# CSB5/XNA_Basecaller

Hardware: NVIDIA B200
Metric: signal samples/sec basecalled (sup@v3.3 XNA) (higher is better)
Workload: dtype fp16

## Files before the change

xna_basecaller_b200/csrc/inproj_gemm.cu:

```cuda
#include <stdlib.h>

#include "xb_common.cuh"
#include "xb_ptx.cuh"
#include "xb_gemm.cuh"
#include "xb_head_epilogue.cuh"
#include "xb_exact_math.h"

using namespace xbptx;

namespace {

#ifdef XB_EXPERIMENTS
#define IP_CLK() clock64()
#else
#define IP_CLK() 0ll
#endif

constexpr int BM = 128, BNI = 64, BK = 64;
constexpr int KB = XB_FEATURES / BK;
constexpr int MAX_COLS = XB_GATES;
constexpr int KPS = 4;
constexpr int SPT = KB / KPS;
enum { IP_GATES = 0, IP_SCORES = 1 };
template <int EPI> struct IPCfg {
    static constexpr int STAGES = EPI == IP_GATES ? 6 : 4;
    static constexpr int SETS = EPI == IP_GATES ? 1 : 2;
    static constexpr int THREADS = (4 + 4 * SETS) * 32;
    static constexpr int STG_BYTES = EPI == IP_GATES ? 32 * (BNI * 2 + 16) : 32 * 81 * 4;
    static constexpr int SMEM_BYTES = STAGES * (KPS * BNI * BK * 2) + 4 * SETS * STG_BYTES + MAX_COLS * 4 + 1024  + 512 ;
};
constexpr int KBLOCK_BYTES = BNI * BK * 2;
constexpr int STAGE_BYTES = KPS * KBLOCK_BYTES;
constexpr int A_COLS = XB_FEATURES / 2;
constexpr int ROW_PITCH = BNI * 2 + 16;

struct IPParams {
    const uint16_t *x;
    const float *bias;
    void *out;
    int M;
    int NT;
    int n_valid, ldo;
    int n_base, expand;
    float scale, blank;
    int exp_out;
    int no_prefetch;
    long long *dbg;
};

template <int NB, bool FULL>
__device__ __forceinline__ void head_stage64(const float (&v)[BNI], uint32_t sr, int e0, int pos0, int ncols, float blank) {
#pragma unroll
    for (int jj = 0; jj < BNI; jj++) {
        if (FULL || jj < ncols) {
            const unsigned u = (unsigned)(e0 + jj);
            const unsigned g = u / NB;
            const uint32_t a = sr + 4u * (uint32_t)(pos0 + jj + (int)g);
            sts_f32(a, v[jj]);
            if (u - g * NB == 0) sts_f32(a - 4u, blank);
        }
    }
}
template <bool FULL>
__device__ __forceinline__ void head_stage64_dyn(const float (&v)[BNI], uint32_t sr, int nb, int e0, int pos0, int ncols, float blank) {
    int e = e0, o = pos0;
#pragma unroll
    for (int jj = 0; jj < BNI; jj++) {
        if (FULL || jj < ncols) {
            if (e == 0) sts_f32(sr + 4u * (uint32_t)(o - 1), blank);
            sts_f32(sr + 4u * (uint32_t)o, v[jj]);
            o++;
            if (++e == nb) { e = 0; o++; }
        }
    }
}

template <bool BF16, int EPI, bool XCP>
__global__ void __launch_bounds__(IPCfg<EPI>::THREADS, 1)
inproj_kernel(const __grid_constant__ CUtensorMap tmW, const __grid_constant__ CUtensorMap tmX, const IPParams p) {
    using X = xb16<BF16>;
    constexpr int STAGES = IPCfg<EPI>::STAGES, STG_BYTES = IPCfg<EPI>::STG_BYTES;
    const int NT = p.NT;
    extern __shared__ uint8_t smem_raw[];
    uint8_t *smem = reinterpret_cast<uint8_t *>((reinterpret_cast<uintptr_t>(smem_raw) + 1023) & ~uintptr_t(1023));
    uint8_t *stgbuf = smem + STAGES * STAGE_BYTES;
    float *sbias = reinterpret_cast<float *>(stgbuf + 4 * IPCfg<EPI>::SETS * STG_BYTES);
    uint64_t *full = reinterpret_cast<uint64_t *>(sbias + MAX_COLS);
    uint64_t *empty = full + STAGES;
    uint64_t *acc_full = empty + STAGES;
    uint64_t *acc_empty = acc_full + 2;
    uint64_t *a_ready = acc_empty + 2;
    uint32_t *tmem_holder = reinterpret_cast<uint32_t *>(a_ready + SPT);

    const int warp = __shfl_sync(0xffffffffu, (int)(threadIdx.x >> 5), 0), lane = threadIdx.x & 31;
    const int ntiles = (p.M + BM - 1) / BM;

    if (warp == 0 && lane == 0) {
        prefetch_tmap(&tmW);
        for (int s = 0; s < STAGES; s++) {
            mbar_init(&full[s], 1);
            mbar_init(&empty[s], 1);
        }
        for (int b = 0; b < 2; b++) {
            mbar_init(&acc_full[b], 1);
            mbar_init(&acc_empty[b], 4);
        }
        for (int ks = 0; ks < SPT; ks++) mbar_init(&a_ready[ks], 4);
        fence_barrier_init();
    }
    if (warp == 2) {
        tmem_alloc(tmem_holder, 512);
        tmem_relinquish();
    }
    for (int i = threadIdx.x; i < NT * BNI; i += IPCfg<EPI>::THREADS) sbias[i] = i < p.n_valid ? p.bias[i] : 0.0f;
    tc_fence_before();
    __syncthreads();
    tc_fence_after();
    const uint32_t tmem_base = *tmem_holder;

    if (warp == 0) {
        if (elect_one()) {
            uint32_t it = 0;
            for (int tile = blockIdx.x; tile < ntiles; tile += gridDim.x) {
                if (XCP)
                    for (int xs = 0; xs < KB / 2; xs++, it++) {
                        const int s = it % STAGES;
                        mbar_wait(&empty[s], ((it / STAGES) & 1) ^ 1);
                        mbar_expect_tx(&full[s], STAGE_BYTES);
                        tma_load_3d(smem + s * STAGE_BYTES, &tmX, &full[s], 0, tile * BM, xs * 2);
                    }
                for (int nt = 0; nt < NT; nt++)
                    for (int ks = 0; ks < SPT; ks++, it++) {
                        const int s = it % STAGES;
                        mbar_wait(&empty[s], ((it / STAGES) & 1) ^ 1);
                        mbar_expect_tx(&full[s], STAGE_BYTES);
                        tma_load_3d(smem + s * STAGE_BYTES, &tmW, &full[s], 0, nt * BNI, ks * KPS);
                    }
            }
        }
    } else if (warp == 1) {
        constexpr uint32_t idesc = umma_idesc_f16(BF16 ? 1u : 0u, BM, BNI);
        uint32_t it = 0, nit = 0, tit = 0;
        long long st_acc = 0, st_full = 0, st_issue = 0, st_a = 0, tt;
        const bool dbg = p.dbg && blockIdx.x == 0;
        for (int tile = blockIdx.x; tile < ntiles; tile += gridDim.x, tit++) {
            if (XCP) {
                tt = IP_CLK();
                for (int xs = 0; xs < KB / 2; xs++, it++) {
                    const int s = it % STAGES;
                    mbar_wait(&full[s], (it / STAGES) & 1);
                    tc_fence_after();
                    if (elect_one()) {
                        const uint64_t sdesc = umma_desc_sw128(smem_u32(smem + s * STAGE_BYTES));
#pragma unroll
                        for (int kk = 0; kk < 8; kk++)
                            tmem_cp_128x256b(tmem_base + (xs * 2) * (BK / 2) + kk * 8,
                                             sdesc + (uint64_t)(((kk >> 2) * (BM * BK * 2) + (kk & 3) * 32) >> 4));
                        mma_commit(&empty[s]);
                    }
                    __syncwarp();
                }
                st_a += IP_CLK() - tt;
            }
            for (int nt = 0; nt < NT; nt++, nit++) {
                const int buf = nit & 1;
                tt = IP_CLK();
                mbar_wait(&acc_empty[buf], ((nit >> 1) & 1) ^ 1);
                tc_fence_after();
                st_acc += IP_CLK() - tt;
                const uint32_t d = tmem_base + A_COLS + buf * BNI;
                for (int ks = 0; ks < SPT; ks++, it++) {
                    const int s = it % STAGES;
                    tt = IP_CLK();
                    mbar_wait(&full[s], (it / STAGES) & 1);
                    tc_fence_after();
                    st_full += IP_CLK() - tt;
                    if (!XCP && nt == 0) {
                        tt = IP_CLK();
                        mbar_wait(&a_ready[ks], tit & 1);
                        tc_fence_after();
                        st_a += IP_CLK() - tt;
                    }
                    tt = IP_CLK();
                    if (elect_one()) {
                        const uint64_t bdesc = umma_desc_sw128(smem_u32(smem + s * STAGE_BYTES));
                        const uint32_t a0 = tmem_base + ks * KPS * (BK / 2);
#pragma unroll
                        for (int kk = 0; kk < KPS * 4; kk++) {
                            const int kc = kk >> 2, k = kk & 3;
                            mma_f16_ts(d, a0 + kk * 8, bdesc + (uint64_t)((kc * KBLOCK_BYTES + k * 32) >> 4), idesc,
                                       (ks | kk) != 0);
                        }
                        mma_commit(&empty[s]);
                        if (ks == SPT - 1) mma_commit(&acc_full[buf]);
                    }
                    __syncwarp();
                    st_issue += IP_CLK() - tt;
                }
            }
        }
        if (dbg && lane == 0) { p.dbg[0] = st_acc; p.dbg[1] = st_full; p.dbg[2] = st_issue; p.dbg[3] = st_a; p.dbg[4] = tit; }
    } else if (warp >= 4) {
        constexpr int SETS = IPCfg<EPI>::SETS;
        const int set = (warp - 4) >> 2;
        const int q = warp & 3, r = q * 32 + lane;
        const uint32_t lane_base = tmem_base + ((uint32_t)(q * 32) << 16);
        uint8_t *stg = stgbuf + (set * 4 + q) * STG_BYTES;
        const uint32_t stg_s = smem_u32(stg);
        uint32_t nit = 0;
        bool pending = false;
        int pend_m0 = 0;

        auto epilogue = [&](int m0, int nt, uint32_t ni) {
            const int buf = ni & 1;
            uint32_t acc[BNI];
            {
                uint32_t a0[32], a1[32];
                tmem_ld_32x32b_x32(lane_base + A_COLS + buf * BNI, a0);
                tmem_ld_32x32b_x32(lane_base + A_COLS + buf * BNI + 32, a1);
                tmem_ld_wait();
#pragma unroll
                for (int i = 0; i < 32; i++) { acc[i] = a0[i]; acc[32 + i] = a1[i]; }
            }
            tc_fence_before();
            __syncwarp();
            if (lane == 0) mbar_arrive(&acc_empty[buf]);
            if constexpr (EPI == IP_GATES) {
                const float *bs = sbias + nt * BNI;
    #pragma unroll
                for (int j = 0; j < BNI / 8; j++) {
                    uint32_t pk[4];
    #pragma unroll
                    for (int e = 0; e < 4; e++)
                        pk[e] = X::pack(__uint_as_float(acc[8 * j + 2 * e]) + bs[8 * j + 2 * e],
                                        __uint_as_float(acc[8 * j + 2 * e + 1]) + bs[8 * j + 2 * e + 1]);
                    sts_v4(stg_s + lane * ROW_PITCH + j * 16, make_uint4(pk[0], pk[1], pk[2], pk[3]));
                }
                __syncwarp();
                const int sub = lane >> 3, l8 = lane & 7;
    #pragma unroll
                for (int rr = 0; rr < 32; rr += 4) {
                    const int mm = m0 + q * 32 + rr + sub;
                    if (mm < p.M)
                        reinterpret_cast<uint4 *>(reinterpret_cast<uint16_t *>(p.out) + (size_t)mm * p.ldo + nt * BNI)[l8] =
                            lds_v4(stg_s + (rr + sub) * ROW_PITCH + l8 * 16);
                }
            } else {
                constexpr int RS = 81;
                float *S = reinterpret_cast<float *>(stg);
// ... 42 lines not shown
                        for (int r = 0; r < 4; r++) {
                            const uint32_t a = sl + (uint32_t)((rr + r) * RS * 4);
                            w[r][0] = k0 ? lds_f32(a) : 0.0f;
                            w[r][1] = k1 ? lds_f32(a + 128) : 0.0f;
                            w[r][2] = k2 ? lds_f32(a + 256) : 0.0f;
                        }
#pragma unroll
                        for (int r = 0; r < 4; r++) {
                            const int mm = m0 + q * 32 + rr + r;
                            if (mm < p.M) {
                                float *o = obase + (size_t)mm * p.ldo;
                                if (k0) o[0] = w[r][0];
                                if (k1) o[32] = w[r][1];
                                if (k2) o[64] = w[r][2];
                            }
                        }
                    }
                    if (dbg) p.dbg[7] += IP_CLK() - te0;
                }
            }
            __syncwarp();
        };

        for (int tile = blockIdx.x; tile < ntiles || pending; tile += gridDim.x) {
            const bool valid = tile < ntiles;
            const int m0 = tile * BM;
            if (pending && ((!XCP && set == 0) || SETS == 1 || (int)((nit - 1) & 1) == set)) {
                mbar_wait(&acc_full[(nit - 1) & 1], ((nit - 1) >> 1) & 1);
                tc_fence_after();
            }
            const long long tl0 = IP_CLK();
            if (!XCP && valid && set == 0) {
                const int sub = lane >> 3, l8 = lane & 7;
                const int mrow0 = m0 + q * 32;
                constexpr int NBK = 2;
                static_assert(KPS == 2 * NBK && KB % KPS == 0, "one a_ready group = two rounds");
                uint4 ldA[NBK][8], ldB[NBK][8];
                auto issue = [&](uint4 (&ld)[NBK][8], int kb0) {
#pragma unroll
                    for (int b = 0; b < NBK; b++)
#pragma unroll
                        for (int i = 0; i < 8; i++) {
                            const int mm = mrow0 + 4 * i + sub;
                            ld[b][i] = (mm < p.M) ? __ldg(reinterpret_cast<const uint4 *>(p.x + (size_t)mm * XB_FEATURES + (kb0 + b) * BK) + l8)
                                                  : make_uint4(0, 0, 0, 0);
                        }
                };
                auto consume = [&](uint4 (&ld)[NBK][8], int kb0) {
#pragma unroll
                    for (int b = 0; b < NBK; b++) {
#pragma unroll
                        for (int i = 0; i < 8; i++)
                            sts_v4(stg_s + (4 * i + sub) * ROW_PITCH + l8 * 16, ld[b][i]);
                        __syncwarp();
                        uint32_t v[32];
#pragma unroll
                        for (int i = 0; i < 8; i++) {
                            const uint4 t4 = lds_v4(stg_s + lane * ROW_PITCH + i * 16);
                            v[4 * i] = t4.x; v[4 * i + 1] = t4.y; v[4 * i + 2] = t4.z; v[4 * i + 3] = t4.w;
                        }
                        __syncwarp();
                        tmem_st_32x32b_x32(lane_base + (kb0 + b) * (BK / 2), v);
                    }
                };
                issue(ldA, 0);
#pragma unroll 1
                for (int kb0 = 0; kb0 < KB; kb0 += KPS) {
                    issue(ldB, kb0 + NBK);
                    consume(ldA, kb0);
                    if (kb0 + KPS < KB) issue(ldA, kb0 + KPS);
                    consume(ldB, kb0 + NBK);
                    tmem_st_wait();
                    tc_fence_before();
                    __syncwarp();
                    if (lane == 0) mbar_arrive(&a_ready[kb0 / KPS]);
                }
            }
            if (p.dbg && blockIdx.x == 0 && warp == 4 && lane == 0) p.dbg[5] += IP_CLK() - tl0;
            for (int nt = -1; nt < (valid ? NT - 1 : 0); nt++) {
                int em0, ent;
                uint32_t eni;
                if (nt < 0) {
                    if (!pending || (SETS > 1 && (int)((nit - 1) & 1) != set)) continue;
                    em0 = pend_m0; ent = NT - 1; eni = nit - 1;
                } else {
                    if (SETS > 1 && (int)(nit & 1) != set) { nit++; continue; }
                    if (nt == (NT > 8 ? NT - 8 : 0) && !p.no_prefetch) {
                        const int mn = m0 + (int)gridDim.x * BM + r;
                        if (mn < p.M) {
                            const char *nx = reinterpret_cast<const char *>(p.x + (size_t)mn * XB_FEATURES);
#pragma unroll
                            for (int i = 0; i < 12; i++) asm volatile("prefetch.global.L2 [%0];" ::"l"(nx + i * 128));
                        }
                    }
                    mbar_wait(&acc_full[nit & 1], (nit >> 1) & 1);
                    tc_fence_after();
                    em0 = m0; ent = nt; eni = nit;
                    nit++;
                }
                epilogue(em0, ent, eni);
            }
            if (valid) {
                nit++;
                pend_m0 = m0;
            }
            pending = valid;
        }
    }
    tc_fence_before();
    __syncthreads();
    if (warp == 2) {
        tc_fence_after();
        tmem_dealloc(tmem_base, 512);
    }
}

}

template <int EPI>
static int ip_launch(xb_handle *h, const void *w, int w_rows, IPParams p, cudaStream_t s) {
    CUtensorMap tmW, tmX;
    if (int rc = xb_make_tmap_hview(h, &tmW, w, w_rows, BNI, KPS)) return rc;
    if (int rc = xb_make_tmap_hview(h, &tmX, p.x, (uint64_t)p.M, BM, 2)) return rc;
    p.NT = w_rows / BNI;
    p.dbg = nullptr;
    p.no_prefetch = 0;
#ifdef XB_EXPERIMENTS
    static const bool regload = getenv("XB_INPROJ_REGLOAD") != nullptr;
    p.no_prefetch = getenv("XB_INPROJ_NOPF") ? 1 : 0;
    if (getenv("XB_INPROJ_DEBUG")) {
        static long long *d = nullptr;
        if (!d) cudaMalloc(&d, 64);
        p.dbg = d;
    }
#endif
    const int ntiles = (p.M + BM - 1) / BM;
    const int grid = ntiles < h->num_sms ? ntiles : h->num_sms;
    constexpr int SMEM_BYTES = IPCfg<EPI>::SMEM_BYTES;
    static bool configured[4][64] = {};
    const int dv = h->device & 63;
    auto go = [&](auto kernel, int slot) -> int {
        if (!configured[slot][dv]) {
            XB_CUDA(h, cudaFuncSetAttribute(kernel, cudaFuncAttributeMaxDynamicSharedMemorySize, SMEM_BYTES));
            configured[slot][dv] = true;
        }
        kernel<<<grid, IPCfg<EPI>::THREADS, SMEM_BYTES, s>>>(tmW, tmX, p);
        return XB_OK;
    };
    int rc;
#ifdef XB_EXPERIMENTS
    if (regload) rc = go(inproj_kernel<false, EPI, false>, 2);
    else
#endif
    rc = go(inproj_kernel<false, EPI, true>, 3);
    if (rc) return rc;
    XB_LAUNCH_CHECK(h);
#ifdef XB_EXPERIMENTS
    if (p.dbg) {
        long long v[8];
        cudaDeviceSynchronize();
        cudaMemcpy(v, p.dbg, sizeof v, cudaMemcpyDeviceToHost);
        fprintf(stderr, "inproj MMA thread of CTA 0: %lld tiles; stall cycles: acc_empty %lld, full %lld, a_ready %lld; issue %lld; x-block load (warp 4) %lld; head epilogue stage %lld, stage+copy %lld\n", v[4], v[0], v[1], v[3], v[2], v[5], v[6], v[7]);
        cudaMemset(p.dbg, 0, 64);
    }
#endif
    return XB_OK;
}

int xb_inproj_launch(xb_handle *h, const void *x, const void *w_ih, const float *bias, void *gates, int M, cudaStream_t s) {
    IPParams p = {};
    p.x = reinterpret_cast<const uint16_t *>(x);
    p.bias = bias;
    p.out = gates;
    p.M = M;
    p.n_valid = XB_GATES; p.ldo = XB_GATES;
    return ip_launch<IP_GATES>(h, w_ih, XB_GATES, p, s);
}

int xb_head_astationary_launch(xb_handle *h, const void *x, const void *w, int w_rows, const float *bias, int head_rows,
                               float *scores, int ldo, int M, int exp_out, cudaStream_t s) {
    XB_REQUIRE(h, w_rows % BNI == 0 && w_rows <= MAX_COLS && head_rows <= w_rows, "head of %d rows unsupported", head_rows);
    IPParams p = {};
    p.x = reinterpret_cast<const uint16_t *>(x);
    p.bias = bias;
    p.out = scores;
// ... 8 lines not shown
```

xna_basecaller_b200/csrc/xb_api.cu:

```cuda
#include <stdarg.h>
#include <stdlib.h>
#include <string.h>

#include "xb_common.cuh"
#include "xb_gemm.cuh"

thread_local std::string xb_global_err;

int xb_fail(xb_handle *h, int code, const char *fmt, ...) {
    char buf[512];
    va_list ap;
    va_start(ap, fmt);
    vsnprintf(buf, sizeof buf, fmt, ap);
    va_end(ap);
    if (h) h->err = buf;
    xb_global_err = buf;
    return code;
}

int xb_conv12_im2col(xb_handle *h, const void *signal, int sig_dtype, int N, int L, cudaStream_t s);
int xb_lstm_recurrence_persistent(xb_handle *h, int layer, void *y_tnc, int T, int N, int reverse, cudaStream_t s, void *save = nullptr);
int xb_inproj_launch(xb_handle *h, const void *x, const void *w_ih, const float *bias, void *gates, int M, cudaStream_t s);
int xb_head_astationary_launch(xb_handle *h, const void *x, const void *w, int w_rows, const float *bias, int head_rows,
                               float *scores, int ldo, int M, int exp_out, cudaStream_t s);
int xb_preprocess_impl(xb_handle *h, const int16_t *raw, const int64_t *read_offset, const int32_t *read_len,
                       const double *scaling, const int32_t *offset, int n_reads, float *out, int32_t *out_len,
                       float *stats, cudaStream_t s);
int xb_ctc_loss_bwd_impl(xb_handle *h, const float *scores, int T, int N, const int32_t *targets, int Lmax,
                         const int32_t *lengths, int normalise, const float *grad_loss, float *alpha_ws, float *grad,
                         cudaStream_t s);
int xb_ctc_loss_impl(xb_handle *h, const float *scores, int T, int N, const int32_t *targets, int Lmax,
                     const int32_t *lengths, int normalise, float *loss, cudaStream_t s);
int xb_stitch_impl(xb_handle *h, const int8_t *rows, int T, const int32_t *chunk_first, const int32_t *chunk_count,
                   const int32_t *read_len, int n_reads, int chunksize, int overlap, int stride, int reverse, int8_t *out,
                   int out_stride, int32_t *out_len, cudaStream_t s);

void xb_train_free(xb_handle *h);
int xb_beam_search_impl(xb_handle *h, const float *scores, const float *beta, int T, int N, int beam_width, float beam_cut,
                        int8_t *seq, int8_t *qstring, int8_t *moves, int32_t *lens, cudaStream_t s);
int xb_onehot_edges(xb_handle *h, const int32_t *edges_nt, int T, int N, int S, float *post, cudaStream_t s);
int xb_gather_chunks_impl(xb_handle *h, const void *signal, int sig_dtype, const int64_t *read_offset,
                          const int32_t *read_len, const int32_t *chunk_read, const int32_t *chunk_start, int n_chunks,
                          int L, float *out, cudaStream_t s);

namespace {
// ... 132 lines not shown
    h->device = device;
    h->max_N = max_N;
    h->max_T = max_T;
    h->n_base = n_base;
    h->state_len = state_len;
    h->C = ipow(n_base, state_len);
    h->NZ = n_base + 1;
    h->flags = flags;
    h->bf16 = (flags & XB_FLAG_BF16) != 0;
    h->num_sms = prop.multiProcessorCount;
    strncpy(h->alphabet, alphabet, sizeof h->alphabet - 1);

    const size_t TN = (size_t)max_T * max_N, S = (size_t)h->C * h->NZ;
    int rc = XB_OK;
#define TRY(x) if (rc == XB_OK) rc = (x)
    const size_t VP = (size_t)((h->C + 31) / 32) * 32 + 4;
    TRY(dev_alloc(h, &h->alpha, (TN + max_N) * VP));
    TRY(dev_alloc(h, &h->bmax, (TN + max_N) * VP));
    TRY(dev_alloc(h, &h->lp, (TN + max_N) * VP));
    TRY(dev_alloc(h, &h->logz, (size_t)max_N));
    TRY(dev_alloc(h, &h->seq_dev, TN));
    TRY(dev_alloc(h, &h->lens_dev, (size_t)max_N));
    if (!(flags & XB_FLAG_NO_ENCODER)) {
        TRY(dev_alloc_bytes(h, &h->c2, TN * XB_CONV3_K * 2));
        TRY(dev_alloc_bytes(h, &h->act0, TN * XB_FEATURES * 2));
        TRY(dev_alloc_bytes(h, &h->act1, TN * XB_FEATURES * 2));
        TRY(dev_alloc_bytes(h, &h->gates, TN * XB_GATES * 2));
        TRY(dev_alloc(h, &h->cstate, (size_t)max_N * XB_FEATURES));
        TRY(dev_alloc(h, &h->scores, TN * S));
        TRY(dev_alloc_bytes(h, &h->signal_dev, TN * XB_STRIDE * sizeof(float)));
    }
#undef TRY
    if (rc != XB_OK) {
        xb_global_err = h->err;
        xb_destroy(h);
        return rc;
    }
    *out = h;
    return XB_OK;
}

int xb_destroy(xb_handle *h) {
    if (!h) return XB_OK;
    cudaSetDevice(h->device);
    void *ptrs[] = {h->conv1_w, h->conv1_b, h->conv2_w, h->conv2_b, h->conv3_w, h->conv3_b, h->head_w, h->head_b, h->c2,
                    h->act0, h->act1, h->gates, h->cstate, h->hzero, h->scores, h->signal_dev, h->seq_dev, h->lens_dev,
// ... 485 lines not shown
```

xna_basecaller_b200/csrc/xb_common.cuh:

```cuda
#pragma once

#include <cuda_runtime.h>
#include <cuda_fp16.h>
#include <cuda_bf16.h>
#include <cuda.h>
#include <stdint.h>
#include <stdio.h>
#include <string>
#include <vector>

#include "../../include/xna_basecaller.h"

#define XB_FEATURES 768
#define XB_GATES (4 * XB_FEATURES)
#define XB_STRIDE 5
#define XB_WINLEN 19
#define XB_C2_CH 16
#define XB_C2_HALO 9
#define XB_CONV3_K 320

struct xb_lstm_weights {
    void *w_ih = nullptr;
    void *w_hh = nullptr;
    float *bias = nullptr;
    void *w_ihT = nullptr;
    void *w_hhT = nullptr;
};

enum { XB_ST_CONV12 = 0, XB_ST_CONV3, XB_ST_INPROJ, XB_ST_LSTM_REC, XB_ST_HEAD, XB_ST_CRF_ALPHA, XB_ST_CRF_BACKWARD,
       XB_ST_CRF_VITERBI, XB_ST_TRAIN_BPTT, XB_ST_TRAIN_TRANSPOSE, XB_ST_TRAIN_WGRAD, XB_ST_TRAIN_XGRAD, XB_ST_TRAIN_HEAD_CONV,
       XB_ST_COUNT };

struct xb_prof_span { int stage; cudaEvent_t a, b; };

struct xb_handle {
    int device = 0;
    bool profiling = false;
    std::vector<xb_prof_span> spans;
    std::vector<cudaEvent_t> event_pool;
    int max_N = 0, max_T = 0;
    int n_base = 0, state_len = 0, C = 0, NZ = 0;
    int flags = 0;
    bool bf16 = false;
    int loaded = 0;
    char alphabet[16] = {0};
    int num_sms = 0;
    int64_t launches = 0;
    std::string err;

    float *conv1_w = nullptr, *conv1_b = nullptr, *conv2_w = nullptr, *conv2_b = nullptr;
    void *conv3_w = nullptr;
    float *conv3_b = nullptr;
    xb_lstm_weights lstm[5];
    void *head_w = nullptr;
    float *head_b = nullptr;
    int head_rows = 0, head_rows_padded = 0;
    float scale = 5.0f, blank_score = 2.0f;
    int expand_blanks = 1;

    void *c2 = nullptr;
    void *act0 = nullptr, *act1 = nullptr;
    void *gates = nullptr;
    float *cstate = nullptr;
    void *hzero = nullptr;
    float *scores = nullptr;
    void *signal_dev = nullptr;
    int8_t *seq_dev = nullptr;
    int32_t *lens_dev = nullptr;
    void *signal_dev2 = nullptr;
// ... 97 lines not shown
```

xna_basecaller_b200/csrc/xb_ptx.cuh:

```cuda
#pragma once
#include <cuda.h>
#include <stdint.h>

namespace xbptx {

__device__ __forceinline__ uint32_t smem_u32(const void *p) { return (uint32_t)__cvta_generic_to_shared(p); }

__device__ __forceinline__ bool elect_one() {
    uint32_t pred;
    asm volatile(
        "{\n\t.reg .pred P;\n\t.reg .b32 R;\n\t"
        "elect.sync R|P, 0xffffffff;\n\t"
        "selp.b32 %0, 1, 0, P;\n\t}"
        : "=r"(pred));
    return pred != 0;
}

__device__ __forceinline__ void mbar_init(uint64_t *bar, uint32_t count) {
    asm volatile("mbarrier.init.shared::cta.b64 [%0], %1;" ::"r"(smem_u32(bar)), "r"(count));
}
__device__ __forceinline__ void fence_barrier_init() { asm volatile("fence.mbarrier_init.release.cluster;" ::: "memory"); }
__device__ __forceinline__ void fence_proxy_async() { asm volatile("fence.proxy.async.shared::cta;" ::: "memory"); }
__device__ __forceinline__ void fence_proxy_async_all() { asm volatile("fence.proxy.async;" ::: "memory"); }
__device__ __forceinline__ void fence_proxy_async_global() { asm volatile("fence.proxy.async.global;" ::: "memory"); }
// ... 51 lines not shown
        "mbarrier.try_wait.parity.shared::cta.b64 P, [%1], %2;\n\t"
        "selp.b32 %0, 1, 0, P;\n\t}"
        : "=r"(ok)
        : "r"(smem_u32(bar)), "r"(parity)
        : "memory");
    return ok != 0;
}
__device__ __forceinline__ bool mbar_test_wait(uint64_t *bar, uint32_t parity) {
    uint32_t ok;
    asm volatile(
        "{\n\t.reg .pred P;\n\t"
        "mbarrier.test_wait.parity.shared::cta.b64 P, [%1], %2;\n\t"
        "selp.b32 %0, 1, 0, P;\n\t}"
        : "=r"(ok)
        : "r"(smem_u32(bar)), "r"(parity)
        : "memory");
    return ok != 0;
}
__device__ __forceinline__ void mbar_wait(uint64_t *bar, uint32_t parity) {
    while (!mbar_try_wait(bar, parity)) {
    }
}

__device__ __forceinline__ void prefetch_tmap(const CUtensorMap *m) {
    asm volatile("prefetch.tensormap [%0];" ::"l"(m) : "memory");
}
__device__ __forceinline__ void tma_load_2d(void *dst, const CUtensorMap *m, uint64_t *bar, int c0, int c1) {
    asm volatile(
        "cp.async.bulk.tensor.2d.shared::cluster.global.mbarrier::complete_tx::bytes [%0], [%1, {%3, %4}], [%2];"
        ::"r"(smem_u32(dst)), "l"(m), "r"(smem_u32(bar)), "r"(c0), "r"(c1)
        : "memory");
}
__device__ __forceinline__ void tma_load_3d(void *dst, const CUtensorMap *m, uint64_t *bar, int c0, int c1, int c2) {
    asm volatile(
        "cp.async.bulk.tensor.3d.shared::cluster.global.mbarrier::complete_tx::bytes [%0], [%1, {%3, %4, %5}], [%2];"
        ::"r"(smem_u32(dst)), "l"(m), "r"(smem_u32(bar)), "r"(c0), "r"(c1), "r"(c2)
        : "memory");
}

__device__ __forceinline__ void tma_store_2d(const CUtensorMap *m, uint32_t src_smem, int c0, int c1) {
    asm volatile("cp.async.bulk.tensor.2d.global.shared::cta.bulk_group [%0, {%2, %3}], [%1];"
                 ::"l"(m), "r"(src_smem), "r"(c0), "r"(c1) : "memory");
}
__device__ __forceinline__ void tma_load_4d(void *dst, const CUtensorMap *m, uint64_t *bar, int c0, int c1, int c2, int c3) {
    asm volatile(
        "cp.async.bulk.tensor.4d.shared::cluster.global.mbarrier::complete_tx::bytes [%0], [%1, {%3, %4, %5, %6}], [%2];"
        ::"r"(smem_u32(dst)), "l"(m), "r"(smem_u32(bar)), "r"(c0), "r"(c1), "r"(c2), "r"(c3)
        : "memory");
}
__device__ __forceinline__ void tma_store_4d(const CUtensorMap *m, uint32_t src_smem, int c0, int c1, int c2, int c3) {
    asm volatile("cp.async.bulk.tensor.4d.global.shared::cta.bulk_group [%0, {%2, %3, %4, %5}], [%1];"
                 ::"l"(m), "r"(src_smem), "r"(c0), "r"(c1), "r"(c2), "r"(c3) : "memory");
}
__device__ __forceinline__ void griddep_launch_dependents() { asm volatile("griddepcontrol.launch_dependents;" ::: "memory"); }
__device__ __forceinline__ void griddep_wait() { asm volatile("griddepcontrol.wait;" ::: "memory"); }
__device__ __forceinline__ void bulk_commit_group() { asm volatile("cp.async.bulk.commit_group;" ::: "memory"); }
__device__ __forceinline__ void bulk_wait_group0() { asm volatile("cp.async.bulk.wait_group 0;" ::: "memory"); }

__device__ __forceinline__ void tmem_alloc(uint32_t *holder_smem, uint32_t ncols) {
    asm volatile("tcgen05.alloc.cta_group::1.sync.aligned.shared::cta.b32 [%0], %1;" ::"r"(smem_u32(holder_smem)), "r"(ncols)
                 : "memory");
}
__device__ __forceinline__ void tmem_relinquish() {
    asm volatile("tcgen05.relinquish_alloc_permit.cta_group::1.sync.aligned;" ::: "memory");
}
__device__ __forceinline__ void tmem_dealloc(uint32_t taddr, uint32_t ncols) {
    asm volatile("tcgen05.dealloc.cta_group::1.sync.aligned.b32 %0, %1;" ::"r"(taddr), "r"(ncols) : "memory");
}
__device__ __forceinline__ void tc_fence_before() { asm volatile("tcgen05.fence::before_thread_sync;" ::: "memory"); }
__device__ __forceinline__ void tc_fence_after() { asm volatile("tcgen05.fence::after_thread_sync;" ::: "memory"); }

__device__ __forceinline__ void mma_f16_ss(uint32_t d_tmem, uint64_t adesc, uint64_t bdesc, uint32_t idesc, uint32_t accumulate) {
    asm volatile(
        "{\n\t.reg .pred p;\n\t"
        "setp.ne.b32 p, %4, 0;\n\t"
        "tcgen05.mma.cta_group::1.kind::f16 [%0], %1, %2, %3, p;\n\t}"
        ::"r"(d_tmem), "l"(adesc), "l"(bdesc), "r"(idesc), "r"(accumulate)
        : "memory");
}
__device__ __forceinline__ void mma_f16_ts(uint32_t d_tmem, uint32_t a_tmem, uint64_t bdesc, uint32_t idesc, uint32_t accumulate) {
    asm volatile(
        "{\n\t.reg .pred p;\n\t"
        "setp.ne.b32 p, %4, 0;\n\t"
        "tcgen05.mma.cta_group::1.kind::f16 [%0], [%1], %2, %3, p;\n\t}"
        ::"r"(d_tmem), "r"(a_tmem), "l"(bdesc), "r"(idesc), "r"(accumulate)
        : "memory");
}
__device__ __forceinline__ void tmem_cp_128x256b(uint32_t taddr, uint64_t sdesc) {
    asm volatile("tcgen05.cp.cta_group::1.128x256b [%0], %1;" ::"r"(taddr), "l"(sdesc) : "memory");
}
__device__ __forceinline__ void mma_commit(uint64_t *bar) {
    asm volatile("tcgen05.commit.cta_group::1.mbarrier::arrive::one.shared::cluster.b64 [%0];" ::"r"(smem_u32(bar)) : "memory");
}

__device__ __forceinline__ void tmem_ld_32x32b_x32(uint32_t taddr, uint32_t (&r)[32]) {
    asm volatile(
        "tcgen05.ld.sync.aligned.32x32b.x32.b32 "
        "{%0, %1, %2, %3, %4, %5, %6, %7, %8, %9, %10, %11, %12, %13, %14, %15, "
        "%16, %17, %18, %19, %20, %21, %22, %23, %24, %25, %26, %27, %28, %29, %30, %31}, [%32];"
        : "=r"(r[0]), "=r"(r[1]), "=r"(r[2]), "=r"(r[3]), "=r"(r[4]), "=r"(r[5]), "=r"(r[6]), "=r"(r[7]), "=r"(r[8]),
          "=r"(r[9]), "=r"(r[10]), "=r"(r[11]), "=r"(r[12]), "=r"(r[13]), "=r"(r[14]), "=r"(r[15]), "=r"(r[16]),
          "=r"(r[17]), "=r"(r[18]), "=r"(r[19]), "=r"(r[20]), "=r"(r[21]), "=r"(r[22]), "=r"(r[23]), "=r"(r[24]),
          "=r"(r[25]), "=r"(r[26]), "=r"(r[27]), "=r"(r[28]), "=r"(r[29]), "=r"(r[30]), "=r"(r[31])
        : "r"(taddr)
        : "memory");
}
__device__ __forceinline__ void tmem_ld_32x32b_x8(uint32_t taddr, uint32_t (&r)[8]) {
    asm volatile("tcgen05.ld.sync.aligned.32x32b.x8.b32 {%0, %1, %2, %3, %4, %5, %6, %7}, [%8];"
                 : "=r"(r[0]), "=r"(r[1]), "=r"(r[2]), "=r"(r[3]), "=r"(r[4]), "=r"(r[5]), "=r"(r[6]), "=r"(r[7])
                 : "r"(taddr)
                 : "memory");
}
__device__ __forceinline__ void tmem_ld_32x32b_x16(uint32_t taddr, uint32_t (&r)[16]) {
    asm volatile(
        "tcgen05.ld.sync.aligned.32x32b.x16.b32 "
// ... 34 lines not shown
```

Baseline: 83.87 million.

## Use 2-CTA cluster tcgen05 MMA pairs for input projection GEMM

Converts the gates input-projection kernel to a two-CTA cluster using cta_group::2 MMAs with M=256, so each CTA loads half the weight tile and weight traffic per output row is halved. TMA loads, barriers, TMEM alloc and commits are routed to the leader CTA, with cluster-scope arrivals. It also removes the register-load (non-XCP) A path so the x block always goes through tcgen05.cp, and adds a startup occupancy query for co-resident pairs. The cost is cluster scheduling constraints, cross-CTA synchronisation and more pipeline stages to keep full.

```diff
diff --git a/xna_basecaller_b200/csrc/inproj_gemm.cu b/xna_basecaller_b200/csrc/inproj_gemm.cu
--- a/xna_basecaller_b200/csrc/inproj_gemm.cu
+++ b/xna_basecaller_b200/csrc/inproj_gemm.cu
@@ -23,14 +23,18 @@
 constexpr int SPT = KB / KPS;
 enum { IP_GATES = 0, IP_SCORES = 1 };
 template <int EPI> struct IPCfg {
-    static constexpr int STAGES = EPI == IP_GATES ? 6 : 4;
+    static constexpr bool PAIR = EPI == IP_GATES;
+    static constexpr int CTAS = PAIR ? 2 : 1;
+    static constexpr int TM = CTAS * BM;
+    static constexpr int WROWS = BNI / CTAS;
+    static constexpr int STAGE_BYTES = KPS * WROWS * BK * 2;
+    static constexpr int XKB = STAGE_BYTES / (BM * BK * 2);
+    static constexpr int STAGES = PAIR ? 12 : 4;
     static constexpr int SETS = EPI == IP_GATES ? 1 : 2;
     static constexpr int THREADS = (4 + 4 * SETS) * 32;
     static constexpr int STG_BYTES = EPI == IP_GATES ? 32 * (BNI * 2 + 16) : 32 * 81 * 4;
-    static constexpr int SMEM_BYTES = STAGES * (KPS * BNI * BK * 2) + 4 * SETS * STG_BYTES + MAX_COLS * 4 + 1024  + 512 ;
+    static constexpr int SMEM_BYTES = STAGES * STAGE_BYTES + 4 * SETS * STG_BYTES + MAX_COLS * 4 + 1024  + 512 ;
 };
-constexpr int KBLOCK_BYTES = BNI * BK * 2;
-constexpr int STAGE_BYTES = KPS * KBLOCK_BYTES;
 constexpr int A_COLS = XB_FEATURES / 2;
 constexpr int ROW_PITCH = BNI * 2 + 16;
 
@@ -75,25 +79,28 @@
     }
 }
 
-template <bool BF16, int EPI, bool XCP>
+template <bool BF16, int EPI>
 __global__ void __launch_bounds__(IPCfg<EPI>::THREADS, 1)
 inproj_kernel(const __grid_constant__ CUtensorMap tmW, const __grid_constant__ CUtensorMap tmX, const IPParams p) {
     using X = xb16<BF16>;
-    constexpr int STAGES = IPCfg<EPI>::STAGES, STG_BYTES = IPCfg<EPI>::STG_BYTES;
+    using C = IPCfg<EPI>;
+    constexpr int STAGES = C::STAGES, STG_BYTES = C::STG_BYTES, STAGE_BYTES = C::STAGE_BYTES, XKB = C::XKB, TM = C::TM;
+    constexpr int CG = C::CTAS;
     const int NT = p.NT;
     extern __shared__ uint8_t smem_raw[];
     uint8_t *smem = reinterpret_cast<uint8_t *>((reinterpret_cast<uintptr_t>(smem_raw) + 1023) & ~uintptr_t(1023));
     uint8_t *stgbuf = smem + STAGES * STAGE_BYTES;
-    float *sbias = reinterpret_cast<float *>(stgbuf + 4 * IPCfg<EPI>::SETS * STG_BYTES);
+    float *sbias = reinterpret_cast<float *>(stgbuf + 4 * C::SETS * STG_BYTES);
     uint64_t *full = reinterpret_cast<uint64_t *>(sbias + MAX_COLS);
     uint64_t *empty = full + STAGES;
     uint64_t *acc_full = empty + STAGES;
     uint64_t *acc_empty = acc_full + 2;
-    uint64_t *a_ready = acc_empty + 2;
-    uint32_t *tmem_holder = reinterpret_cast<uint32_t *>(a_ready + SPT);
+    uint32_t *tmem_holder = reinterpret_cast<uint32_t *>(acc_empty + 2);
 
     const int warp = __shfl_sync(0xffffffffu, (int)(threadIdx.x >> 5), 0), lane = threadIdx.x & 31;
-    const int ntiles = (p.M + BM - 1) / BM;
+    const uint32_t rank = C::PAIR ? cluster_ctarank() : 0;
+    const int unit = blockIdx.x / CG, units = gridDim.x / CG;
+    const int ntiles = (p.M + TM - 1) / TM;
 
     if (warp == 0 && lane == 0) {
         prefetch_tmap(&tmW);
@@ -103,65 +110,69 @@
         }
         for (int b = 0; b < 2; b++) {
             mbar_init(&acc_full[b], 1);
-            mbar_init(&acc_empty[b], 4);
-        }
-        for (int ks = 0; ks < SPT; ks++) mbar_init(&a_ready[ks], 4);
+            mbar_init(&acc_empty[b], 4 * CG);
+        }
         fence_barrier_init();
     }
     if (warp == 2) {
-        tmem_alloc(tmem_holder, 512);
-        tmem_relinquish();
-    }
-    for (int i = threadIdx.x; i < NT * BNI; i += IPCfg<EPI>::THREADS) sbias[i] = i < p.n_valid ? p.bias[i] : 0.0f;
+        tmem_alloc<CG>(tmem_holder, 512);
+        tmem_relinquish<CG>();
+    }
+    for (int i = threadIdx.x; i < NT * BNI; i += C::THREADS) sbias[i] = i < p.n_valid ? p.bias[i] : 0.0f;
     tc_fence_before();
-    __syncthreads();
+    if (C::PAIR) cluster_sync();
+    else __syncthreads();
     tc_fence_after();
     const uint32_t tmem_base = *tmem_holder;
 
     if (warp == 0) {
         if (elect_one()) {
+            const uint32_t full_bar = C::PAIR ? mapa_shared(full, 0) : 0;
+            auto load = [&](int s, const CUtensorMap *m, int c1, int c2) {
+                if (rank == 0) mbar_expect_tx(&full[s], CG * STAGE_BYTES);
+                if constexpr (C::PAIR) tma_load_3d_pair(smem + s * STAGE_BYTES, m, full_bar + s * 8, 0, c1, c2);
+                else tma_load_3d(smem + s * STAGE_BYTES, m, &full[s], 0, c1, c2);
+            };
             uint32_t it = 0;
-            for (int tile = blockIdx.x; tile < ntiles; tile += gridDim.x) {
-                if (XCP)
-                    for (int xs = 0; xs < KB / 2; xs++, it++) {
-                        const int s = it % STAGES;
-                        mbar_wait(&empty[s], ((it / STAGES) & 1) ^ 1);
-                        mbar_expect_tx(&full[s], STAGE_BYTES);
-                        tma_load_3d(smem + s * STAGE_BYTES, &tmX, &full[s], 0, tile * BM, xs * 2);
-                    }
+            for (int tile = unit; tile < ntiles; tile += units) {
+                for (int xs = 0; xs < KB / XKB; xs++, it++) {
+                    const int s = it % STAGES;
+                    mbar_wait(&empty[s], ((it / STAGES) & 1) ^ 1);
+                    load(s, &tmX, tile * TM + (int)rank * BM, xs * XKB);
+                }
                 for (int nt = 0; nt < NT; nt++)
                     for (int ks = 0; ks < SPT; ks++, it++) {
                         const int s = it % STAGES;
                         mbar_wait(&empty[s], ((it / STAGES) & 1) ^ 1);
-                        mbar_expect_tx(&full[s], STAGE_BYTES);
-                        tma_load_3d(smem + s * STAGE_BYTES, &tmW, &full[s], 0, nt * BNI, ks * KPS);
-                    }
-            }
-        }
-    } else if (warp == 1) {
-        constexpr uint32_t idesc = umma_idesc_f16(BF16 ? 1u : 0u, BM, BNI);
+                        load(s, &tmW, nt * BNI + (int)rank * C::WROWS, ks * KPS);
+                    }
+            }
+            if (C::PAIR)
+                for (int i = 0; i < STAGES; i++, it++) mbar_wait(&empty[it % STAGES], ((it / STAGES) & 1) ^ 1);
+        }
+    } else if (warp == 1 && rank == 0) {
+        constexpr uint32_t idesc = umma_idesc_f16(BF16 ? 1u : 0u, TM, BNI);
+        constexpr int KBLOCK_BYTES = C::WROWS * BK * 2;
         uint32_t it = 0, nit = 0, tit = 0;
         long long st_acc = 0, st_full = 0, st_issue = 0, st_a = 0, tt;
         const bool dbg = p.dbg && blockIdx.x == 0;
-        for (int tile = blockIdx.x; tile < ntiles; tile += gridDim.x, tit++) {
-            if (XCP) {
-                tt = IP_CLK();
-                for (int xs = 0; xs < KB / 2; xs++, it++) {
-                    const int s = it % STAGES;
-                    mbar_wait(&full[s], (it / STAGES) & 1);
-                    tc_fence_after();
-                    if (elect_one()) {
-                        const uint64_t sdesc = umma_desc_sw128(smem_u32(smem + s * STAGE_BYTES));
-#pragma unroll
-                        for (int kk = 0; kk < 8; kk++)
-                            tmem_cp_128x256b(tmem_base + (xs * 2) * (BK / 2) + kk * 8,
+        for (int tile = unit; tile < ntiles; tile += units, tit++) {
+            tt = IP_CLK();
+            for (int xs = 0; xs < KB / XKB; xs++, it++) {
+                const int s = it % STAGES;
+                mbar_wait(&full[s], (it / STAGES) & 1);
+                tc_fence_after();
+                if (elect_one()) {
+                    const uint64_t sdesc = umma_desc_sw128(smem_u32(smem + s * STAGE_BYTES));
+#pragma unroll
+                    for (int kk = 0; kk < 4 * XKB; kk++)
+                        tmem_cp_128x256b<CG>(tmem_base + (xs * XKB) * (BK / 2) + kk * 8,
                                              sdesc + (uint64_t)(((kk >> 2) * (BM * BK * 2) + (kk & 3) * 32) >> 4));
-                        mma_commit(&empty[s]);
-                    }
-                    __syncwarp();
-                }
-                st_a += IP_CLK() - tt;
-            }
+                    mma_commit<CG>(&empty[s]);
+                }
+                __syncwarp();
+            }
+            st_a += IP_CLK() - tt;
             for (int nt = 0; nt < NT; nt++, nit++) {
                 const int buf = nit & 1;
                 tt = IP_CLK();
@@ -175,12 +186,6 @@
                     mbar_wait(&full[s], (it / STAGES) & 1);
                     tc_fence_after();
                     st_full += IP_CLK() - tt;
-                    if (!XCP && nt == 0) {
-                        tt = IP_CLK();
-                        mbar_wait(&a_ready[ks], tit & 1);
-                        tc_fence_after();
-                        st_a += IP_CLK() - tt;
-                    }
                     tt = IP_CLK();
                     if (elect_one()) {
                         const uint64_t bdesc = umma_desc_sw128(smem_u32(smem + s * STAGE_BYTES));
@@ -188,11 +193,11 @@
 #pragma unroll
                         for (int kk = 0; kk < KPS * 4; kk++) {
                             const int kc = kk >> 2, k = kk & 3;
-                            mma_f16_ts(d, a0 + kk * 8, bdesc + (uint64_t)((kc * KBLOCK_BYTES + k * 32) >> 4), idesc,
-                                       (ks | kk) != 0);
+                            mma_f16_ts<CG>(d, a0 + kk * 8, bdesc + (uint64_t)((kc * KBLOCK_BYTES + k * 32) >> 4), idesc,
+                                           (ks | kk) != 0);
                         }
-                        mma_commit(&empty[s]);
-                        if (ks == SPT - 1) mma_commit(&acc_full[buf]);
+                        mma_commit<CG>(&empty[s]);
+                        if (ks == SPT - 1) mma_commit<CG>(&acc_full[buf]);
                     }
                     __syncwarp();
                     st_issue += IP_CLK() - tt;
@@ -207,6 +212,7 @@
         const uint32_t lane_base = tmem_base + ((uint32_t)(q * 32) << 16);
         uint8_t *stg = stgbuf + (set * 4 + q) * STG_BYTES;
         const uint32_t stg_s = smem_u32(stg);
+        const uint32_t acc_empty_bar = C::PAIR ? mapa_shared(acc_empty, 0) : 0;
         uint32_t nit = 0;
         bool pending = false;
         int pend_m0 = 0;
@@ -224,7 +230,10 @@
             }
             tc_fence_before();
             __syncwarp();
-            if (lane == 0) mbar_arrive(&acc_empty[buf]);
+            if (lane == 0) {
+                if constexpr (C::PAIR) mbar_arrive_cluster(acc_empty_bar + buf * 8);
+                else mbar_arrive(&acc_empty[buf]);
+            }
             if constexpr (EPI == IP_GATES) {
                 const float *bs = sbias + nt * BNI;
     #pragma unroll
@@ -313,61 +322,13 @@
             __syncwarp();
         };
 
-        for (int tile = blockIdx.x; tile < ntiles || pending; tile += gridDim.x) {
+        for (int tile = unit; tile < ntiles || pending; tile += units) {
             const bool valid = tile < ntiles;
-            const int m0 = tile * BM;
-            if (pending && ((!XCP && set == 0) || SETS == 1 || (int)((nit - 1) & 1) == set)) {
+            const int m0 = tile * TM + (int)rank * BM;
+            if (pending && (SETS == 1 || (int)((nit - 1) & 1) == set)) {
                 mbar_wait(&acc_full[(nit - 1) & 1], ((nit - 1) >> 1) & 1);
                 tc_fence_after();
             }
-            const long long tl0 = IP_CLK();
-            if (!XCP && valid && set == 0) {
-                const int sub = lane >> 3, l8 = lane & 7;
-                const int mrow0 = m0 + q * 32;
-                constexpr int NBK = 2;
-                static_assert(KPS == 2 * NBK && KB % KPS == 0, "one a_ready group = two rounds");
-                uint4 ldA[NBK][8], ldB[NBK][8];
-                auto issue = [&](uint4 (&ld)[NBK][8], int kb0) {
-#pragma unroll
-                    for (int b = 0; b < NBK; b++)
-#pragma unroll
-                        for (int i = 0; i < 8; i++) {
-                            const int mm = mrow0 + 4 * i + sub;
-                            ld[b][i] = (mm < p.M) ? __ldg(reinterpret_cast<const uint4 *>(p.x + (size_t)mm * XB_FEATURES + (kb0 + b) * BK) + l8)
-                                                  : make_uint4(0, 0, 0, 0);
-                        }
-                };
-                auto consume = [&](uint4 (&ld)[NBK][8], int kb0) {
-#pragma unroll
-                    for (int b = 0; b < NBK; b++) {
-#pragma unroll
-                        for (int i = 0; i < 8; i++)
-                            sts_v4(stg_s + (4 * i + sub) * ROW_PITCH + l8 * 16, ld[b][i]);
-                        __syncwarp();
-                        uint32_t v[32];
-#pragma unroll
-                        for (int i = 0; i < 8; i++) {
-                            const uint4 t4 = lds_v4(stg_s + lane * ROW_PITCH + i * 16);
-                            v[4 * i] = t4.x; v[4 * i + 1] = t4.y; v[4 * i + 2] = t4.z; v[4 * i + 3] = t4.w;
-                        }
-                        __syncwarp();
-                        tmem_st_32x32b_x32(lane_base + (kb0 + b) * (BK / 2), v);
-                    }
-                };
-                issue(ldA, 0);
-#pragma unroll 1
-                for (int kb0 = 0; kb0 < KB; kb0 += KPS) {
-                    issue(ldB, kb0 + NBK);
-                    consume(ldA, kb0);
-                    if (kb0 + KPS < KB) issue(ldA, kb0 + KPS);
-                    consume(ldB, kb0 + NBK);
-                    tmem_st_wait();
-                    tc_fence_before();
-                    __syncwarp();
-                    if (lane == 0) mbar_arrive(&a_ready[kb0 / KPS]);
-                }
-            }
-            if (p.dbg && blockIdx.x == 0 && warp == 4 && lane == 0) p.dbg[5] += IP_CLK() - tl0;
             for (int nt = -1; nt < (valid ? NT - 1 : 0); nt++) {
                 int em0, ent;
                 uint32_t eni;
@@ -377,7 +338,7 @@
                 } else {
                     if (SETS > 1 && (int)(nit & 1) != set) { nit++; continue; }
                     if (nt == (NT > 8 ? NT - 8 : 0) && !p.no_prefetch) {
-                        const int mn = m0 + (int)gridDim.x * BM + r;
+                        const int mn = m0 + units * TM + r;
                         if (mn < p.M) {
                             const char *nx = reinterpret_cast<const char *>(p.x + (size_t)mn * XB_FEATURES);
 #pragma unroll
@@ -399,25 +360,55 @@
         }
     }
     tc_fence_before();
-    __syncthreads();
+    if (C::PAIR) cluster_sync();
+    else __syncthreads();
     if (warp == 2) {
         tc_fence_after();
-        tmem_dealloc(tmem_base, 512);
-    }
-}
-
+        tmem_dealloc<CG>(tmem_base, 512);
+    }
+}
+
+}
+
+template <int EPI>
+static int ip_configure(xb_handle *h) {
+    static bool configured[64] = {};
+    const int dv = h->device & 63;
+    if (!configured[dv]) {
+        XB_CUDA(h, cudaFuncSetAttribute(inproj_kernel<false, EPI>, cudaFuncAttributeMaxDynamicSharedMemorySize, IPCfg<EPI>::SMEM_BYTES));
+        configured[dv] = true;
+    }
+    return XB_OK;
+}
+
+int xb_inproj_query_pairs(xb_handle *h) {
+    if (int rc = ip_configure<IP_GATES>(h)) return rc;
+    cudaLaunchConfig_t cfg = {};
+    cudaLaunchAttribute attr[1];
+    attr[0].id = cudaLaunchAttributeClusterDimension;
+    attr[0].val.clusterDim.x = 2; attr[0].val.clusterDim.y = 1; attr[0].val.clusterDim.z = 1;
+    cfg.gridDim = dim3(2 * (h->num_sms / 2));
+    cfg.blockDim = dim3(IPCfg<IP_GATES>::THREADS);
+    cfg.dynamicSmemBytes = IPCfg<IP_GATES>::SMEM_BYTES;
+    cfg.attrs = attr;
+    cfg.numAttrs = 1;
+    int n = 0;
+    XB_CUDA(h, cudaOccupancyMaxActiveClusters(&n, inproj_kernel<false, IP_GATES>, &cfg));
+    if (n < 1) return xb_fail(h, XB_ERR_UNSUPPORTED, "the input projection needs co-resident CTA pairs, the device fits none");
+    h->inproj_pairs = n;
+    return XB_OK;
 }
 
 template <int EPI>
 static int ip_launch(xb_handle *h, const void *w, int w_rows, IPParams p, cudaStream_t s) {
+    using C = IPCfg<EPI>;
     CUtensorMap tmW, tmX;
-    if (int rc = xb_make_tmap_hview(h, &tmW, w, w_rows, BNI, KPS)) return rc;
-    if (int rc = xb_make_tmap_hview(h, &tmX, p.x, (uint64_t)p.M, BM, 2)) return rc;
+    if (int rc = xb_make_tmap_hview(h, &tmW, w, w_rows, C::WROWS, KPS)) return rc;
+    if (int rc = xb_make_tmap_hview(h, &tmX, p.x, (uint64_t)p.M, BM, C::XKB)) return rc;
     p.NT = w_rows / BNI;
     p.dbg = nullptr;
     p.no_prefetch = 0;
 #ifdef XB_EXPERIMENTS
-    static const bool regload = getenv("XB_INPROJ_REGLOAD") != nullptr;
     p.no_prefetch = getenv("XB_INPROJ_NOPF") ? 1 : 0;
     if (getenv("XB_INPROJ_DEBUG")) {
         static long long *d = nullptr;
@@ -425,33 +416,27 @@
         p.dbg = d;
     }
 #endif
-    const int ntiles = (p.M + BM - 1) / BM;
-    const int grid = ntiles < h->num_sms ? ntiles : h->num_sms;
-    constexpr int SMEM_BYTES = IPCfg<EPI>::SMEM_BYTES;
-    static bool configured[4][64] = {};
-    const int dv = h->device & 63;
-    auto go = [&](auto kernel, int slot) -> int {
-        if (!configured[slot][dv]) {
-            XB_CUDA(h, cudaFuncSetAttribute(kernel, cudaFuncAttributeMaxDynamicSharedMemorySize, SMEM_BYTES));
-            configured[slot][dv] = true;
-        }
-        kernel<<<grid, IPCfg<EPI>::THREADS, SMEM_BYTES, s>>>(tmW, tmX, p);
-        return XB_OK;
-    };
-    int rc;
-#ifdef XB_EXPERIMENTS
-    if (regload) rc = go(inproj_kernel<false, EPI, false>, 2);
-    else
-#endif
-    rc = go(inproj_kernel<false, EPI, true>, 3);
-    if (rc) return rc;
+    if (int rc = ip_configure<EPI>(h)) return rc;
+    const int ntiles = (p.M + C::TM - 1) / C::TM;
+    const int units = C::PAIR ? h->inproj_pairs : h->num_sms;
+    cudaLaunchConfig_t cfg = {};
+    cudaLaunchAttribute attr[1];
+    attr[0].id = cudaLaunchAttributeClusterDimension;
+    attr[0].val.clusterDim.x = C::CTAS; attr[0].val.clusterDim.y = 1; attr[0].val.clusterDim.z = 1;
+    cfg.gridDim = dim3(C::CTAS * (ntiles < units ? ntiles : units));
+    cfg.blockDim = dim3(C::THREADS);
+    cfg.dynamicSmemBytes = C::SMEM_BYTES;
+    cfg.stream = s;
+    cfg.attrs = attr;
+    cfg.numAttrs = C::PAIR ? 1 : 0;
+    XB_CUDA(h, cudaLaunchKernelEx(&cfg, inproj_kernel<false, EPI>, tmW, tmX, p));
     XB_LAUNCH_CHECK(h);
 #ifdef XB_EXPERIMENTS
     if (p.dbg) {
         long long v[8];
         cudaDeviceSynchronize();
         cudaMemcpy(v, p.dbg, sizeof v, cudaMemcpyDeviceToHost);
-        fprintf(stderr, "inproj MMA thread of CTA 0: %lld tiles; stall cycles: acc_empty %lld, full %lld, a_ready %lld; issue %lld; x-block load (warp 4) %lld; head epilogue stage %lld, stage+copy %lld\n", v[4], v[0], v[1], v[3], v[2], v[5], v[6], v[7]);
+        fprintf(stderr, "inproj MMA thread of CTA 0: %lld tiles; stall cycles: acc_empty %lld, full %lld, x copy %lld; issue %lld; head epilogue stage %lld, stage+copy %lld\n", v[4], v[0], v[1], v[3], v[2], v[6], v[7]);
         cudaMemset(p.dbg, 0, 64);
     }
 #endif
diff --git a/xna_basecaller_b200/csrc/xb_api.cu b/xna_basecaller_b200/csrc/xb_api.cu
--- a/xna_basecaller_b200/csrc/xb_api.cu
+++ b/xna_basecaller_b200/csrc/xb_api.cu
@@ -21,6 +21,7 @@
 int xb_conv12_im2col(xb_handle *h, const void *signal, int sig_dtype, int N, int L, cudaStream_t s);
 int xb_lstm_recurrence_persistent(xb_handle *h, int layer, void *y_tnc, int T, int N, int reverse, cudaStream_t s, void *save = nullptr);
 int xb_inproj_launch(xb_handle *h, const void *x, const void *w_ih, const float *bias, void *gates, int M, cudaStream_t s);
+int xb_inproj_query_pairs(xb_handle *h);
 int xb_head_astationary_launch(xb_handle *h, const void *x, const void *w, int w_rows, const float *bias, int head_rows,
                                float *scores, int ldo, int M, int exp_out, cudaStream_t s);
 int xb_preprocess_impl(xb_handle *h, const int16_t *raw, const int64_t *read_offset, const int32_t *read_len,
@@ -199,6 +200,7 @@
     TRY(dev_alloc(h, &h->seq_dev, TN));
     TRY(dev_alloc(h, &h->lens_dev, (size_t)max_N));
     if (!(flags & XB_FLAG_NO_ENCODER)) {
+        TRY(xb_inproj_query_pairs(h));
         TRY(dev_alloc_bytes(h, &h->c2, TN * XB_CONV3_K * 2));
         TRY(dev_alloc_bytes(h, &h->act0, TN * XB_FEATURES * 2));
         TRY(dev_alloc_bytes(h, &h->act1, TN * XB_FEATURES * 2));
diff --git a/xna_basecaller_b200/csrc/xb_common.cuh b/xna_basecaller_b200/csrc/xb_common.cuh
--- a/xna_basecaller_b200/csrc/xb_common.cuh
+++ b/xna_basecaller_b200/csrc/xb_common.cuh
@@ -45,6 +45,7 @@
     int loaded = 0;
     char alphabet[16] = {0};
     int num_sms = 0;
+    int inproj_pairs = 0;
     int64_t launches = 0;
     std::string err;
 
diff --git a/xna_basecaller_b200/csrc/xb_ptx.cuh b/xna_basecaller_b200/csrc/xb_ptx.cuh
--- a/xna_basecaller_b200/csrc/xb_ptx.cuh
+++ b/xna_basecaller_b200/csrc/xb_ptx.cuh
@@ -97,6 +97,23 @@
     }
 }
 
+__device__ __forceinline__ uint32_t cluster_ctarank() {
+    uint32_t r;
+    asm volatile("mov.u32 %0, %%cluster_ctarank;" : "=r"(r));
+    return r;
+}
+__device__ __forceinline__ void cluster_sync() {
+    asm volatile("barrier.cluster.arrive.release.aligned;\n\tbarrier.cluster.wait.acquire.aligned;" ::: "memory");
+}
+__device__ __forceinline__ uint32_t mapa_shared(const void *p, uint32_t rank) {
+    uint32_t r;
+    asm volatile("mapa.shared::cluster.u32 %0, %1, %2;" : "=r"(r) : "r"(smem_u32(p)), "r"(rank));
+    return r;
+}
+__device__ __forceinline__ void mbar_arrive_cluster(uint32_t bar_cluster) {
+    asm volatile("mbarrier.arrive.shared::cluster.b64 _, [%0];" ::"r"(bar_cluster) : "memory");
+}
+
 __device__ __forceinline__ void prefetch_tmap(const CUtensorMap *m) {
     asm volatile("prefetch.tensormap [%0];" ::"l"(m) : "memory");
 }
@@ -110,6 +127,13 @@
     asm volatile(
         "cp.async.bulk.tensor.3d.shared::cluster.global.mbarrier::complete_tx::bytes [%0], [%1, {%3, %4, %5}], [%2];"
         ::"r"(smem_u32(dst)), "l"(m), "r"(smem_u32(bar)), "r"(c0), "r"(c1), "r"(c2)
+        : "memory");
+}
+
+__device__ __forceinline__ void tma_load_3d_pair(void *dst, const CUtensorMap *m, uint32_t bar_cluster, int c0, int c1, int c2) {
+    asm volatile(
+        "cp.async.bulk.tensor.3d.cta_group::2.shared::cluster.global.mbarrier::complete_tx::bytes [%0], [%1, {%3, %4, %5}], [%2];"
+        ::"r"(smem_u32(dst)), "l"(m), "r"(bar_cluster), "r"(c0), "r"(c1), "r"(c2)
         : "memory");
 }
 
@@ -132,15 +156,24 @@
 __device__ __forceinline__ void bulk_commit_group() { asm volatile("cp.async.bulk.commit_group;" ::: "memory"); }
 __device__ __forceinline__ void bulk_wait_group0() { asm volatile("cp.async.bulk.wait_group 0;" ::: "memory"); }
 
+template <int CG = 1>
 __device__ __forceinline__ void tmem_alloc(uint32_t *holder_smem, uint32_t ncols) {
-    asm volatile("tcgen05.alloc.cta_group::1.sync.aligned.shared::cta.b32 [%0], %1;" ::"r"(smem_u32(holder_smem)), "r"(ncols)
-                 : "memory");
-}
+    if constexpr (CG == 2)
+        asm volatile("tcgen05.alloc.cta_group::2.sync.aligned.shared::cta.b32 [%0], %1;" ::"r"(smem_u32(holder_smem)), "r"(ncols)
+                     : "memory");
+    else
+        asm volatile("tcgen05.alloc.cta_group::1.sync.aligned.shared::cta.b32 [%0], %1;" ::"r"(smem_u32(holder_smem)), "r"(ncols)
+                     : "memory");
+}
+template <int CG = 1>
 __device__ __forceinline__ void tmem_relinquish() {
-    asm volatile("tcgen05.relinquish_alloc_permit.cta_group::1.sync.aligned;" ::: "memory");
-}
+    if constexpr (CG == 2) asm volatile("tcgen05.relinquish_alloc_permit.cta_group::2.sync.aligned;" ::: "memory");
+    else asm volatile("tcgen05.relinquish_alloc_permit.cta_group::1.sync.aligned;" ::: "memory");
+}
+template <int CG = 1>
 __device__ __forceinline__ void tmem_dealloc(uint32_t taddr, uint32_t ncols) {
-    asm volatile("tcgen05.dealloc.cta_group::1.sync.aligned.b32 %0, %1;" ::"r"(taddr), "r"(ncols) : "memory");
+    if constexpr (CG == 2) asm volatile("tcgen05.dealloc.cta_group::2.sync.aligned.b32 %0, %1;" ::"r"(taddr), "r"(ncols) : "memory");
+    else asm volatile("tcgen05.dealloc.cta_group::1.sync.aligned.b32 %0, %1;" ::"r"(taddr), "r"(ncols) : "memory");
 }
 __device__ __forceinline__ void tc_fence_before() { asm volatile("tcgen05.fence::before_thread_sync;" ::: "memory"); }
 __device__ __forceinline__ void tc_fence_after() { asm volatile("tcgen05.fence::after_thread_sync;" ::: "memory"); }
@@ -153,19 +186,35 @@
         ::"r"(d_tmem), "l"(adesc), "l"(bdesc), "r"(idesc), "r"(accumulate)
         : "memory");
 }
+template <int CG = 1>
 __device__ __forceinline__ void mma_f16_ts(uint32_t d_tmem, uint32_t a_tmem, uint64_t bdesc, uint32_t idesc, uint32_t accumulate) {
-    asm volatile(
-        "{\n\t.reg .pred p;\n\t"
-        "setp.ne.b32 p, %4, 0;\n\t"
-        "tcgen05.mma.cta_group::1.kind::f16 [%0], [%1], %2, %3, p;\n\t}"
-        ::"r"(d_tmem), "r"(a_tmem), "l"(bdesc), "r"(idesc), "r"(accumulate)
-        : "memory");
-}
+    if constexpr (CG == 2)
+        asm volatile(
+            "{\n\t.reg .pred p;\n\t"
+            "setp.ne.b32 p, %4, 0;\n\t"
+            "tcgen05.mma.cta_group::2.kind::f16 [%0], [%1], %2, %3, p;\n\t}"
+            ::"r"(d_tmem), "r"(a_tmem), "l"(bdesc), "r"(idesc), "r"(accumulate)
+            : "memory");
+    else
+        asm volatile(
+            "{\n\t.reg .pred p;\n\t"
+            "setp.ne.b32 p, %4, 0;\n\t"
+            "tcgen05.mma.cta_group::1.kind::f16 [%0], [%1], %2, %3, p;\n\t}"
+            ::"r"(d_tmem), "r"(a_tmem), "l"(bdesc), "r"(idesc), "r"(accumulate)
+            : "memory");
+}
+template <int CG = 1>
 __device__ __forceinline__ void tmem_cp_128x256b(uint32_t taddr, uint64_t sdesc) {
-    asm volatile("tcgen05.cp.cta_group::1.128x256b [%0], %1;" ::"r"(taddr), "l"(sdesc) : "memory");
-}
+    if constexpr (CG == 2) asm volatile("tcgen05.cp.cta_group::2.128x256b [%0], %1;" ::"r"(taddr), "l"(sdesc) : "memory");
+    else asm volatile("tcgen05.cp.cta_group::1.128x256b [%0], %1;" ::"r"(taddr), "l"(sdesc) : "memory");
+}
+template <int CG = 1>
 __device__ __forceinline__ void mma_commit(uint64_t *bar) {
-    asm volatile("tcgen05.commit.cta_group::1.mbarrier::arrive::one.shared::cluster.b64 [%0];" ::"r"(smem_u32(bar)) : "memory");
+    if constexpr (CG == 2)
+        asm volatile("tcgen05.commit.cta_group::2.mbarrier::arrive::one.shared::cluster.multicast::cluster.b64 [%0], %1;"
+                     ::"r"(smem_u32(bar)), "h"((uint16_t)0x3) : "memory");
+    else
+        asm volatile("tcgen05.commit.cta_group::1.mbarrier::arrive::one.shared::cluster.b64 [%0];" ::"r"(smem_u32(bar)) : "memory");
 }
 
 __device__ __forceinline__ void tmem_ld_32x32b_x32(uint32_t taddr, uint32_t (&r)[32]) {
```

Result: faster. 86.10 million (median of 6 runs) (+2.7%).
